# IXarea/LittleGAN

Measured on AMD Instinct MI355X. Metric: 128x128 CelebA-shaped images/sec (G+D+Adj step), higher is better.
Workload: dtype bf16; 1 GPU; C3: 128x128x3 synthetic CelebA, batch 256/GPU, bf16 MFMA conv/transposed-conv + Adjuster branch; global_batch=256, per_gpu_batch=256, image=128, cond_dim=40, parallelism=dp1, launch=eager launches

## Files before the change

### include/littlegan_hip.h

```cpp
#ifndef LITTLEGAN_HIP_H
#define LITTLEGAN_HIP_H
#include <stddef.h>

#ifdef __cplusplus
extern "C" {
#endif

#define LG_ABI_VERSION 1
#define LG_OK 0
#define LG_ERR_ARG (-1)
#define LG_ERR_LAUNCH (-2)
#define LG_ERR_UNSUPPORTED (-3)
#define LG_DT_F32 0
#define LG_DT_BF16 1

int lg_abi_version(void);
const char* lg_last_error(void);
const char* lg_last_kernel(void);
int lg_clear_kernel(void);

size_t lg_conv_pack_bytes(int cb, int cs, int dtype);
int lg_conv_pack(const float* w, void* pack, int cb, int cs, int dtype, void* stream);

int lg_conv2d_s2_fwd(const float* x, const void* pack, const float* bias, float* y, int B, int Hs, int Ws, int cb,
// ... 65 lines not shown
                               int B, void* stream);
int lg_instnorm_leaky_apply_z16_p(const void* z16, const void* partials, int nparts, const float* gamma, const float* beta,
                                  float* stats, const void* skip, int skip_is_bf16, float* y, void* y16, int B, long long L,
                                  int post_leaky, float alpha, void* stream);
int lg_instnorm_leaky_apply(const float* x, const float* stats, const float* skip, float* y, void* y16, int B,
                            long long L, int pre_leaky, int post_leaky, float alpha, void* stream);
int lg_instnorm_leaky_bwd(const float* x, const float* stats, const void* g, int g_is_bf16, float* dx, void* dx16,
                          float* dgamma, float* dbeta, void* workspace, size_t ws_bytes, int B, long long L,
                          int pre_leaky, int post_leaky, float alpha, int accumulate, void* stream);
size_t lg_instnorm_bwd_db_workspace_bytes(int B, long long L, int C);
int lg_instnorm_leaky_bwd_db(const float* x, const float* stats, const void* g, int g_is_bf16, float* dx, void* dx16,
                             float* dgamma, float* dbeta, float* db, int C, void* workspace, size_t ws_bytes, int B,
                             long long L, int pre_leaky, int post_leaky, float alpha, int accumulate, void* stream);
int lg_instnorm_leaky_apply_z16(const void* z16, const float* stats, const void* skip, int skip_is_bf16, float* y, void* y16,
                                int B, long long L, int pre_leaky, int post_leaky, float alpha, void* stream);
int lg_instnorm_leaky_bwd_z16(const void* z16, const float* stats, const void* g, int g_is_bf16, float* dx, void* dx16,
                              float* dgamma, float* dbeta, float* db, int C, void* workspace, size_t ws_bytes, int B,
                              long long L, int pre_leaky, int post_leaky, float alpha, int accumulate, void* stream);
int lg_instnorm_leaky_bwd_z16_p(const void* z16, const float* stats, const void* g, int g_is_bf16, float* dx, void* dx16,
                                float* dgamma, float* dbeta, float* db, int C, const void* partials, int nparts_in,
                                void* workspace, size_t ws_bytes, int B, long long L, int pre_leaky, int post_leaky, float alpha,
                                int accumulate, void* stream);
int lg_conv2d_s2_dgrad_nf(const void* dy16, const void* pack, void* dx16, int B, int Hs, int Ws, int cb, int cs,
                          const void* z16, const float* stats, float alpha, void* part, size_t part_bytes, int* nparts,
                          void* stream);
int lg_convT_s2_dgrad_nf(const void* dy16, const void* pack, void* dx16, int B, int Hs, int Ws, int cb, int cs,
                         const void* z16, const float* stats, float alpha, void* part, size_t part_bytes, int* nparts,
                         void* stream);

int lg_convT_s2_dgrad_bn_supported(int B, int Hs, int Ws, int cb, int cs);
int lg_convT_s2_dgrad_bn(const void* z16, const void* g16, const float* coef, float alpha, const void* pack, void* dx16,
                         int B, int Hs, int Ws, int cb, int cs, const void* zl16, const float* stats_l, float alpha_l,
                         void* part, size_t part_bytes, int* nparts, void* stream);
int lg_instnorm_bwd_coef(const float* stats, const void* partials, int nparts, float* coef, int B, long long L, void* stream);

int lg_dropout_key(long long* key, unsigned long long seed, unsigned long long key_offset, void* stream);
int lg_dropout_mask(const long long* key, int call, int level, int r0, int B, long long L, float rate, unsigned char* keep,
                    void* stream);
int lg_instnorm_leaky_apply_drop(const float* x, const float* stats, float* y, void* y16, int B, long long L, float alpha,
                                 const long long* key, int call, int level, int r0, float rate, void* stream);
int lg_instnorm_leaky_apply_z16_drop(const void* z16, const float* stats, float* y, void* y16, int B, long long L, float alpha,
                                     const long long* key, int call, int level, int r0, float rate, void* stream);
int lg_instnorm_leaky_apply_z16_p_drop(const void* z16, const void* partials, int nparts, const float* gamma, const float* beta,
                                       float* stats, float* y, void* y16, int B, long long L, float alpha, const long long* key,
                                       int call, int level, int r0, float rate, void* stream);
int lg_instnorm_leaky_bwd_drop(const float* x, const float* stats, const void* g, int g_is_bf16, float* dx, void* dx16,
                               float* dgamma, float* dbeta, float* db, int C, void* workspace, size_t ws_bytes, int B,
                               long long L, float alpha, int accumulate, const long long* key, int call, int level, int r0,
                               float rate, void* stream);
int lg_instnorm_leaky_bwd_z16_drop(const void* z16, const float* stats, const void* g, int g_is_bf16, float* dx, void* dx16,
                                   float* dgamma, float* dbeta, float* db, int C, const void* partials, int nparts_in,
                                   void* workspace, size_t ws_bytes, int B, long long L, float alpha, int accumulate,
                                   const long long* key, int call, int level, int r0, float rate, void* stream);

int lg_convT_s1_tanh_bwd_nf(const float* x, const void* x16, const float* dpre, const void* pack, void* dx16, float* dw,
                            float* db, void* workspace, size_t ws_bytes, int B, int H, int W, int cb, int cs, int accumulate,
                            int dtype, const void* z16, const float* stats, float alpha, void* part, size_t part_bytes,
                            int* nparts, void* stream);

int lg_dense_fwd(const float* x, const float* w, const float* bias, float* y, int B, int K, int N, void* stream);
int lg_dense_wgrad(const float* x, const float* dy, float* dw, float* db, int B, int K, int N, int accumulate,
                   void* stream);
int lg_dense_dgrad(const float* dy, const float* w, float* dx, int B, int K, int N, void* stream);
int lg_concat_cols(const float* a, int ka, const float* c, int kc, float* out, int B, void* stream);
int lg_adj_conditions(const float* first, const float* second, float* t, float* u, int B, int c, void* stream);
size_t lg_heads_fwd_workspace_bytes(int B, int K, int c);
// ... 80 lines not shown
```

### littlegan_amd/_lib.py

```python
from __future__ import annotations

import ctypes as C
import os

_HERE = os.path.dirname(os.path.abspath(__file__))
LIB_PATH = os.path.join(_HERE, "liblittlegan_hip.so")

DT_F32, DT_BF16 = 0, 1

P, I, L, F, Z = C.c_void_p, C.c_int, C.c_longlong, C.c_float, C.c_size_t

SIGNATURES = {
    "lg_abi_version": (I, []),
    "lg_last_error": (C.c_char_p, []),
    "lg_conv_pack_bytes": (Z, [I, I, I]),
    "lg_conv_pack": (I, [P, P, I, I, I, P]),
    "lg_conv2d_s2_fwd": (I, [P, P, P, P, I, I, I, I, I, I, P]),
    "lg_conv_stats_workspace_bytes": (Z, [I, I, I, I, I]),
    "lg_conv_fwd_stats_fused": (I, [I, I, I, I, I, I, I]),
    "lg_conv2d_s2_fwd_stats": (I, [P, P, P, P, P, P, I, I, I, I, I, I, P, Z, P, P]),
    "lg_conv2d_s2_dgrad_m16": (I, [P, P, P, P, P, I, I, I, I, I, I, P]),
    "lg_conv2d_s2_wgrad_m16": (I, [P, P, P, P, P, P, Z, I, I, I, I, I, I, I, P]),
    "lg_conv2d_s2_dgrad": (I, [P, P, P, I, I, I, I, I, I, P]),
    "lg_conv2d_s2_wgrad": (I, [P, P, P, P, Z, I, I, I, I, I, I, I, P]),
# ... 8 lines not shown
    "lg_convT_s1_tanh_bwd": (I, [P, P, P, P, P, P, P, Z, I, I, I, I, I, I, I, P]),
    "lg_convT_s1_bwd_workspace_bytes": (Z, [I, I, I, I, I, I]),
    "lg_n3_m16_supported": (I, [I, I, I, I, I]),
    "lg_convT_s1_tanh_fwd_m16": (I, [P, P, P, P, P, I, I, I, I, I, I, P]),
    "lg_conv2d_s2_fwd_stats_zn_supported": (I, [I, I, I, I, I, I]),
    "lg_conv2d_s2_fwd_stats_zn": (I, [P, P, F, P, P, P, I, I, I, I, I, I, P, Z, P, P]),
    "lg_convT_s1_tanh_fwd_z16_supported": (I, [I, I, I, I, I]),
    "lg_convT_s1_tanh_fwd_z16": (I, [P, P, F, P, P, P, I, I, I, I, I, I, P]),
    "lg_convT_s1_tanh_bwd_m16": (I, [P, P, P, P, P, P, P, P, P, Z, I, I, I, I, I, I, I, P]),
    "lg_bias_grad_workspace_bytes": (Z, [L, I]),
    "lg_bias_grad": (I, [P, P, P, Z, L, I, I, P]),
    "lg_bias_grad_m16": (I, [P, P, P, P, Z, L, I, I, P]),
    "lg_conv_halo_supported": (I, [I, I, I, I, I, I, I]),
    "lg_instnorm_workspace_bytes": (Z, [I, L]),
    "lg_instnorm_stats_stride": (I, []),
    "lg_instnorm_leaky_stats": (I, [P, P, P, P, P, Z, I, L, I, F, P]),
    "lg_instnorm_leaky_stats_z16": (I, [P, P, P, P, P, Z, I, L, I, F, P, P]),
    "lg_instnorm_stats_finalize": (I, [P, I, P, P, P, I, P]),
    "lg_instnorm_leaky_apply": (I, [P, P, P, P, P, I, L, I, I, F, P]),
    "lg_instnorm_leaky_bwd": (I, [P, P, P, I, P, P, P, P, P, Z, I, L, I, I, F, I, P]),
    "lg_instnorm_bwd_db_workspace_bytes": (Z, [I, L, I]),
    "lg_instnorm_leaky_bwd_db": (I, [P, P, P, I, P, P, P, P, P, I, P, Z, I, L, I, I, F, I, P]),
    "lg_last_kernel": (C.c_char_p, []),
    "lg_clear_kernel": (I, []),
    "lg_instnorm_leaky_apply_z16": (I, [P, P, P, I, P, P, I, L, I, I, F, P]),
    "lg_instnorm_leaky_apply_z16_p": (I, [P, P, I, P, P, P, P, I, P, P, I, L, I, F, P]),
    "lg_instnorm_leaky_bwd_z16": (I, [P, P, P, I, P, P, P, P, P, I, P, Z, I, L, I, I, F, I, P]),
    "lg_instnorm_leaky_bwd_z16_p": (I, [P, P, P, I, P, P, P, P, P, I, P, I, P, Z, I, L, I, I, F, I, P]),
    "lg_conv2d_s2_dgrad_nf": (I, [P, P, P, I, I, I, I, I, P, P, F, P, Z, P, P]),
    "lg_convT_s2_dgrad_nf": (I, [P, P, P, I, I, I, I, I, P, P, F, P, Z, P, P]),
    "lg_convT_s2_dgrad_bn_supported": (I, [I, I, I, I, I]),
    "lg_convT_s2_dgrad_bn": (I, [P, P, P, F, P, P, I, I, I, I, I, P, P, F, P, Z, P, P]),
    "lg_instnorm_bwd_coef": (I, [P, P, I, P, I, L, P]),
    "lg_dropout_key": (I, [P, L, L, P]),
    "lg_dropout_mask": (I, [P, I, I, I, I, L, F, P, P]),
    "lg_instnorm_leaky_apply_drop": (I, [P, P, P, P, I, L, F, P, I, I, I, F, P]),
    "lg_instnorm_leaky_apply_z16_drop": (I, [P, P, P, P, I, L, F, P, I, I, I, F, P]),
    "lg_instnorm_leaky_apply_z16_p_drop": (I, [P, P, I, P, P, P, P, P, I, L, F, P, I, I, I, F, P]),
    "lg_instnorm_leaky_bwd_drop": (I, [P, P, P, I, P, P, P, P, P, I, P, Z, I, L, F, I, P, I, I, I, F, P]),
    "lg_instnorm_leaky_bwd_z16_drop": (I, [P, P, P, I, P, P, P, P, P, I, P, I, P, Z, I, L, F, I, P, I, I, I, F, P]),
    "lg_convT_s1_tanh_bwd_nf": (I, [P, P, P, P, P, P, P, P, Z, I, I, I, I, I, I, I, P, P, F, P, Z, P, P]),
    "lg_dense_fwd": (I, [P, P, P, P, I, I, I, P]),
    "lg_dense_wgrad": (I, [P, P, P, P, I, I, I, I, P]),
    "lg_dense_dgrad": (I, [P, P, P, I, I, I, P]),
    "lg_concat_cols": (I, [P, I, P, I, P, I, P]),
    "lg_adj_conditions": (I, [P, P, P, P, I, I, P]),
    "lg_heads_fwd_workspace_bytes": (Z, [I, I, I]),
    "lg_heads_fwd": (I, [P, P, P, P, P, P, P, Z, I, I, I, P]),
    "lg_heads_dgrad": (I, [P, P, P, P, I, I, I, P]),
    "lg_heads_wgrad": (I, [P, P, P, P, P, P, I, I, I, I, P]),
    "lg_bce_heads_loss_fwd_bwd": (I, [P, P, F, F, F, P, P, I, I, I, P]),
    "lg_l1_workspace_bytes": (Z, []),
    "lg_l1_tanh_loss_fwd_bwd": (I, [P, P, P, P, P, P, Z, L, F, I, P]),
    "lg_clip_adam_update": (I, [P, P, P, P, L, P, F, F, F, F, F, F, P]),
    "lg_adam_advance": (I, [P, F, F, P]),
    "lg_axpby": (I, [P, P, F, F, L, P]),
    "lg_philox4x32": (I, [P, I, L, L, P]),
    "lg_randn": (I, [P, L, F, F, L, L, P]),
    "lg_augment_workspace_bytes": (Z, [I]),
    "lg_augment": (I, [P, P, I, I, I, P, F, F, F, F, L, L, P, Z, P]),
    "lg_fid_stats_workspace_bytes": (Z, [L, I]),
    "lg_fid_stats": (I, [P, L, I, P, P, P, Z, P]),
    "lg_fid_accum": (I, [P, L, I, P, P, P, P]),
    "lg_fid_finalize": (I, [P, P, P, L, I, P, P, P]),
    "lg_fid_gemm": (I, [P, P, P, I, P, P]),
    "lg_fid_distance_workspace_bytes": (Z, [I]),
# ... 65 lines not shown
```

### littlegan_amd/csrc/capi.hip

```cpp
#include <stdarg.h>
#include <stdio.h>
#include <stdlib.h>
#include "lg_common.h"
#include "../../include/littlegan_hip.h"

static thread_local char g_err[512] = "";

extern "C" void lg_set_error(const char* fmt, ...) {
  va_list ap;
  va_start(ap, fmt);
  vsnprintf(g_err, sizeof(g_err), fmt, ap);
  va_end(ap);
}
extern "C" const char* lg_last_error(void) { return g_err; }
static thread_local const char* g_kernel = "";
extern "C" void lg_note_kernel(const char* name) { g_kernel = name ? name : ""; }
extern "C" const char* lg_last_kernel(void) { return g_kernel; }
extern "C" int lg_clear_kernel(void) { g_kernel = ""; return LG_OK; }
extern "C" int lg_abi_version(void) { return LG_ABI_VERSION; }

extern "C" int lg_conv_igemm(int mode, int dtype, const float* src, const void* wpack, const float* bias, float* out,
                             int B, int Hm, int Wm, int Cs, int N, int act, int pstride, int ppad, void* stream);
extern "C" int lg_conv_igemm_ex(int mode, int dtype, const float* src, const void* src16, const void* wpack,
                                const float* bias, float* out, void* out16, int B, int Hm, int Wm, int Cs, int N, int act,
// ... 161 lines not shown
extern "C" int lg_convT_s2_dgrad_nf(const void* dy16, const void* pack, void* dx16, int B, int Hs, int Ws, int cb, int cs,
                                    const void* z16, const float* stats, float alpha, void* part, size_t part_bytes,
                                    int* nparts, void* stream) {
  LG_CHECK_ARG(dy16 && pack && dx16 && nparts, "lg_convT_s2_dgrad_nf: null pointer");
  *nparts = 0;
  if (cb != 3 && z16 && stats && part) {
    LgNormFuse nf{(const __bf16*)z16, stats, (double*)part, alpha, 0};
    const int rc = lg_conv_down3_nf_try(dy16, pack, nullptr, dx16, B, Hs, Ws, cb, cs, nullptr, 0, nparts, &nf, part_bytes, stream);
    if (rc != LG_ERR_UNSUPPORTED) return rc;
    *nparts = 0;
  }
  return lg_convT_s2_dgrad_m16(nullptr, dy16, pack, nullptr, dx16, B, Hs, Ws, cb, cs, LG_DT_BF16, stream);
}

extern "C" int lg_conv_down3_bn_supported(int B, int Hm, int Wm, int Cs, int N);
extern "C" int lg_conv_down3_bn_try(const void* z16, const void* g16, const float* bcoef, float alpha, const void* wpack, void* out16,
                                    int B, int Hm, int Wm, int Cs, int N, int* nparts_out, const LgNormFuse* nf, size_t nf_bytes,
                                    void* stream);
extern "C" int lg_convT_s2_dgrad_bn_supported(int B, int Hs, int Ws, int cb, int cs) {
  return cb != 3 ? lg_conv_down3_bn_supported(B, Hs, Ws, cb, cs) : 0;
}
extern "C" int lg_convT_s2_dgrad_bn(const void* z16, const void* g16, const float* coef, float alpha, const void* pack, void* dx16,
                                    int B, int Hs, int Ws, int cb, int cs, const void* zl16, const float* stats_l, float alpha_l,
                                    void* part, size_t part_bytes, int* nparts, void* stream) {
  LG_CHECK_ARG(z16 && g16 && coef && pack && dx16 && zl16 && stats_l && part && nparts, "lg_convT_s2_dgrad_bn: null pointer");
  *nparts = 0;
  LgNormFuse nf{(const __bf16*)zl16, stats_l, (double*)part, alpha_l, 0};
  const int rc = lg_conv_down3_bn_try(z16, g16, coef, alpha, pack, dx16, B, Hs, Ws, cb, cs, nparts, &nf, part_bytes, stream);
  if (rc == LG_ERR_UNSUPPORTED) lg_set_error("lg_convT_s2_dgrad_bn: shape B=%d %dx%d cb=%d cs=%d has no backward-normalising kernel "
                                             "(see lg_convT_s2_dgrad_bn_supported)", B, Hs, Ws, cb, cs);
  return rc;
}

extern "C" int lg_conv2d_s2_wgrad_m16(const float* x, const void* x16, const float* dy, const void* dy16, float* dw,
                                      void* workspace, size_t ws_bytes, int B, int Hs, int Ws, int cb, int cs,
                                      int accumulate, int dtype, void* stream) {
  return lg_conv_wgrad_m16(x, x16, dy, dy16, dw, workspace, ws_bytes, B, Hs, Ws, cb, cs, 2, 1, accumulate, dtype, stream);
}
extern "C" int lg_convT_s2_wgrad_m16(const float* x, const void* x16, const float* dy, const void* dy16, float* dw,
                                     void* workspace, size_t ws_bytes, int B, int Hs, int Ws, int cb, int cs,
                                     int accumulate, int dtype, void* stream) {
  return lg_conv_wgrad_m16(dy, dy16, x, x16, dw, workspace, ws_bytes, B, Hs, Ws, cb, cs, 2, 1, accumulate, dtype, stream);
}
extern "C" int lg_conv2d_s2_dgrad(const float* dy, const void* pack, float* dx, int B, int Hs, int Ws, int cb, int cs,
                                  int dtype, void* stream) {
  return run_up(dy, pack, nullptr, dx, B, Hs, Ws, cb, cs, dtype, stream);
}
extern "C" int lg_conv2d_s2_wgrad(const float* x, const float* dy, float* dw, void* workspace, size_t ws_bytes, int B,
                                  int Hs, int Ws, int cb, int cs, int accumulate, int dtype, void* stream) {
  return lg_conv_wgrad(x, dy, dw, workspace, ws_bytes, B, Hs, Ws, cb, cs, 2, 1, accumulate, dtype, stream);
}
extern "C" int lg_convT_s2_fwd(const float* x, const void* pack, const float* bias, float* y, int B, int Hs, int Ws,
                               int cb, int cs, int dtype, void* stream) {
  return run_up(x, pack, bias, y, B, Hs, Ws, cb, cs, dtype, stream);
}
extern "C" int lg_convT_s2_dgrad(const float* dy, const void* pack, float* dx, int B, int Hs, int Ws, int cb, int cs,
                                 int dtype, void* stream) {
  return run_down(dy, pack, nullptr, dx, B, Hs, Ws, cb, cs, dtype, stream);
}
extern "C" int lg_convT_s2_wgrad(const float* x, const float* dy, float* dw, void* workspace, size_t ws_bytes, int B,
                                 int Hs, int Ws, int cb, int cs, int accumulate, int dtype, void* stream) {
  return lg_conv_wgrad(dy, x, dw, workspace, ws_bytes, B, Hs, Ws, cb, cs, 2, 1, accumulate, dtype, stream);
}

extern "C" int lg_n3_m16_supported(int H, int W, int cb, int cs, int dtype) {
  return (dtype == LG_DT_BF16 && cb == 3 && lg_n3_enabled() && lg_n3_p16_supported(H, W, cs)) ? 1 : 0;
// ... 138 lines not shown
```

### littlegan_amd/csrc/n3_pgemm.hip

```cpp
#include <type_traits>
#include "lg_common.h"

#ifndef LG_P16_DBG
#define LG_P16_DBG 0
#endif
namespace {

constexpr int TS = 16;
constexpr int PR = 17;

__device__ __forceinline__ bf16x8 cvt8(const float* p) {
  const f32x4 a = *reinterpret_cast<const f32x4*>(p), b = *reinterpret_cast<const f32x4*>(p + 4);
  bf16x8 v;
  v[0] = (__bf16)a[0]; v[1] = (__bf16)a[1]; v[2] = (__bf16)a[2]; v[3] = (__bf16)a[3];
  v[4] = (__bf16)b[0]; v[5] = (__bf16)b[1]; v[6] = (__bf16)b[2]; v[7] = (__bf16)b[3];
  return v;
}
__device__ __forceinline__ bf16x8 zero8() {
  return __builtin_bit_cast(bf16x8, u32x4{0u, 0u, 0u, 0u});
}

template <int C>
__device__ __forceinline__ void load_bfrags(const float* __restrict__ w, int lane, bf16x8 (&bf)[5][C / 32]) {
  const int n = lane & 15, g = lane >> 4;
// ... 25 lines not shown
#pragma unroll
    for (int kh = 0; kh < KH; ++kh)
      af[i][kh] = ok ? *reinterpret_cast<const bf16x8*>(x16 + ((long long)(n * H + sy) * W + sx) * C + kh * 32 + g * 8) : zero8();
  }
  load_bfrags<C>(w, lane, bf);

  const int ly = threadIdx.x / TS, lx = threadIdx.x % TS;
  float acc[3] = {bias[0], bias[1], bias[2]};
#pragma unroll
  for (int ky = 0; ky < 5; ++ky) {
#pragma unroll
    for (int i = 0; i < MTW; ++i) {
      const int mt = wid + 4 * i;
      if (mt < NMT) {
        f32x4 c = {0.f, 0.f, 0.f, 0.f};
#pragma unroll
        for (int kh = 0; kh < KH; ++kh) c = __builtin_amdgcn_mfma_f32_16x16x32_bf16(af[i][kh], bf[ky][kh], c, 0, 0, 0);
#pragma unroll
        for (int e = 0; e < 4; ++e) sP[(mt * 16 + 4 * g + e) * PR + r] = c[e];
      }
    }
    __syncthreads();
#pragma unroll
    for (int kx = 0; kx < 5; ++kx) {
      const float* pp = sP + ((ly + 4 - ky) * HS + (lx + 4 - kx)) * PR + kx * 3;
      acc[0] += pp[0]; acc[1] += pp[1]; acc[2] += pp[2];
    }
    __syncthreads();
  }
  float* o = y + ((long long)(n * H + y0 + ly) * W + x0 + lx) * 3;
  o[0] = tanhf(acc[0]); o[1] = tanhf(acc[1]); o[2] = tanhf(acc[2]);
}

template <int C>
__global__ __launch_bounds__(256, 1) void up_p16_kernel(const __bf16* __restrict__ src16, const float* __restrict__ w,
                                                     float* __restrict__ out, int B, int H, int W) {
  constexpr int HS = TS + 2, NQ = HS * HS, NMT = (NQ + 15) / 16, MTW = (NMT + 3) / 4, KH = C / 32;
  __shared__ float sP[NMT * 16 * PR];
  const int lane = threadIdx.x & 63, wid = threadIdx.x >> 6, r = lane & 15, g = lane >> 4;
  const int tpx = W / TS, tpi = tpx * (H / TS), ntiles = B * tpi, G = gridDim.x;

  bf16x8 bf[5][KH];
  load_bfrags<C>(w, lane, bf);
  auto load_af = [&](int t, bf16x8 (&af)[MTW][KH]) {
    const int n = t / tpi, tt = t - n * tpi;
    const int y0 = (tt / tpx) * TS, x0 = (tt % tpx) * TS;
#pragma unroll
    for (int i = 0; i < MTW; ++i) {
      const int mt = wid + 4 * i, q = mt * 16 + r;
      const int sy = y0 - 1 + q / HS, sx = x0 - 1 + q % HS;
      const bool ok = q < NQ && (unsigned)sy < (unsigned)H && (unsigned)sx < (unsigned)W;
#pragma unroll
      for (int kh = 0; kh < KH; ++kh)
        af[i][kh] = (ok && !(LG_P16_DBG & 64)) ? *reinterpret_cast<const bf16x8*>(src16 + ((long long)(n * H + sy) * W + sx) * C + kh * 32 + g * 8) : zero8();
    }
  };
  const int ly = threadIdx.x / TS, lx = threadIdx.x % TS;
  auto compute = [&](int t, const bf16x8 (&af)[MTW][KH]) {
    const int n = t / tpi, tt = t - n * tpi;
    const int y0 = (tt / tpx) * TS, x0 = (tt % tpx) * TS;
    float acc[4][3];
#pragma unroll
    for (int k = 0; k < 4; ++k) { acc[k][0] = 0.f; acc[k][1] = 0.f; acc[k][2] = 0.f; }
#pragma unroll
    for (int ky = 0; ky < 5; ++ky) {
#pragma unroll
      for (int i = 0; i < MTW; ++i) {
        const int mt = wid + 4 * i;
        if (mt < NMT) {
          f32x4 c = {0.f, 0.f, 0.f, 0.f};
#pragma unroll
          for (int kh = 0; kh < KH; ++kh) c = __builtin_amdgcn_mfma_f32_16x16x32_bf16(af[i][kh], bf[ky][kh], c, 0, 0, 0);
#pragma unroll
          for (int e = 0; e < 4; ++e) {
            if constexpr (!(LG_P16_DBG & 32)) sP[(mt * 16 + 4 * g + e) * PR + r] = c[e];
            else if (c[e] == 12345.f) sP[(mt * 16 + 4 * g + e) * PR + r] = c[e];
          }
        }
      }
      if constexpr (!(LG_P16_DBG & 128)) __syncthreads();
      const int py = 1 - (ky & 1), dy = (py + 1 - ky) / 2;
#pragma unroll
      for (int kx = 0; kx < ((LG_P16_DBG & 16) ? 1 : 5); ++kx) {
        const int px = 1 - (kx & 1), dx = (px + 1 - kx) / 2;
        const float* pp = sP + ((ly + 1 + dy) * HS + (lx + 1 + dx)) * PR + kx * 3;
        acc[py * 2 + px][0] += pp[0]; acc[py * 2 + px][1] += pp[1]; acc[py * 2 + px][2] += pp[2];
      }
      if constexpr (!(LG_P16_DBG & 128)) __syncthreads();
    }
    const int yq = y0 + ly, xq = x0 + lx;
#pragma unroll
    for (int py = 0; py < 2; ++py) {
      float* o = out + ((long long)(n * 2 * H + 2 * yq + py) * 2 * W + 2 * xq) * 3;
#pragma unroll
      for (int px = 0; px < 2; ++px)
#pragma unroll
        for (int co = 0; co < 3; ++co) o[px * 3 + co] = acc[py * 2 + px][co];
    }
  };
  bf16x8 afA[MTW][KH], afB[MTW][KH];
  int t = blockIdx.x;
  if (t < ntiles) load_af(t, afA);
  for (; t < ntiles; t += 2 * G) {
    if (t + G < ntiles) load_af(t + G, afB);
    compute(t, afA);
    if (t + G < ntiles) {
      if (t + 2 * G < ntiles) load_af(t + 2 * G, afA);
      compute(t + G, afB);
    }
  }
}


template <int S, int N, bool OUT16, bool STATS, bool FUSE = false>
__global__ __launch_bounds__(256, 4) void patch_p16_kernel(const float* __restrict__ src, const float* __restrict__ w,
                                                        const float* __restrict__ bias, float* __restrict__ out,
                                                        __bf16* __restrict__ out16, double* __restrict__ spart, int B,
                                                        int H, int W, int pad, LgNormFuse nf = LgNormFuse{}) {
  static_assert(!FUSE || (OUT16 && !STATS), "norm-backward sums: bf16 data-gradient form only");
  constexpr bool CSPLIT = N == 64;
  constexpr int NWC = CSPLIT ? N / 2 : N;
  constexpr int NT = NWC / 16, HSIDE = S * (TS - 1) + 5, PW = (HSIDE + 2) & ~1, TROWS = HSIDE + 1, NKS = 4;
  constexpr int MTW = CSPLIT ? TS / 2 : TS / 4;
  constexpr bool HAS_BIAS = S == 2;
  __shared__ __attribute__((aligned(16))) bf16x4 tile[TROWS * PW];
  __shared__ __attribute__((aligned(16))) float cst[4][16 * NWC];
  __shared__ double sred[40];
  const int lane = threadIdx.x & 63, wid = __builtin_amdgcn_readfirstlane(threadIdx.x >> 6), r = lane & 15, g = lane >> 4;
  const int tpx = W / TS, tpi = tpx * (H / TS), ntiles = B * tpi;
  const int Hs = S * H, Ws = S * W;
  const int chw = CSPLIT ? (wid & 1) : 0, rw = CSPLIT ? (wid >> 1) : wid;

  bf16x8 bf[NKS][NT];
#pragma unroll
  for (int ks = 0; ks < NKS; ++ks)
#pragma unroll
    for (int nt = 0; nt < NT; ++nt) {
      bf16x8 v;
#pragma unroll
      for (int j = 0; j < 8; ++j) {
        const int kp = 32 * ks + 8 * g + j, ky = kp / 24, rem = kp - 24 * ky, kx = rem >> 2, c4 = rem & 3;
// ... 160 lines not shown

}

static int patch_grid(int ntiles, int per_cu) {
  static int cus = 0;
  if (!cus) {
    int dev = 0;
    hipDeviceProp_t pr;
    cus = 256;
    if (hipGetDevice(&dev) == hipSuccess && hipGetDeviceProperties(&pr, dev) == hipSuccess && pr.multiProcessorCount > 0) cus = pr.multiProcessorCount;
  }
  const int nb = per_cu * (cus < lg_grid_cus() ? cus : lg_grid_cus());
  return ntiles < nb ? ntiles : nb;
}

extern "C" int lg_n3_p16_supported(int H, int W, int C) { return (H % TS == 0 && W % TS == 0 && (C == 32 || C == 64)) ? 1 : 0; }

extern "C" int lg_n3_s1t_fwd_p16_try(const void* x16, const float* w, const float* bias, float* y, int B, int H, int W,
                                     int C, void* stream) {
  if (!lg_n3_p16_supported(H, W, C) || !x16 || !w || !bias) return LG_ERR_UNSUPPORTED;
  hipStream_t st = (hipStream_t)stream;
  const dim3 grid(B * (H / TS) * (W / TS));
  if (C == 32) hipLaunchKernelGGL(s1t_fwd_p16_kernel<32>, grid, dim3(256), 0, st, (const __bf16*)x16, w, bias, y, B, H, W);
  else hipLaunchKernelGGL(s1t_fwd_p16_kernel<64>, grid, dim3(256), 0, st, (const __bf16*)x16, w, bias, y, B, H, W);
  LG_CHECK_LAUNCH("lg_n3_s1t_fwd_p16");
  lg_note_kernel("s1t_fwd_p16_kernel");
  return LG_OK;
}

extern "C" int lg_n3_up_p16_try(const void* src16, const float* w, float* out, int B, int H, int W, int C, void* stream) {
  if (!lg_n3_p16_supported(H, W, C) || !src16 || !w) return LG_ERR_UNSUPPORTED;
  hipStream_t st = (hipStream_t)stream;
  const dim3 grid(patch_grid(B * (H / TS) * (W / TS), 2));
  if (C == 32) hipLaunchKernelGGL(up_p16_kernel<32>, grid, dim3(256), 0, st, (const __bf16*)src16, w, out, B, H, W);
  else hipLaunchKernelGGL(up_p16_kernel<64>, grid, dim3(256), 0, st, (const __bf16*)src16, w, out, B, H, W);
  LG_CHECK_LAUNCH("lg_n3_up_p16");
  lg_note_kernel("up_p16_kernel");
  return LG_OK;
}

extern "C" int lg_n3_conv1_p16_supported(int H, int W, int N) { return (H % TS == 0 && W % TS == 0 && N == 64) ? 1 : 0; }

extern "C" int lg_n3_conv1_fwd_p16_try(const float* img, const float* w, const float* bias, float* z, void* z16, int B, int H,
                                       int W, int N, void* spart, size_t spart_bytes, int* nparts, void* stream) {
  if (nparts) *nparts = 0;
  if (H % TS || W % TS || N != 64 || !img || !w || (!z && !z16)) return LG_ERR_UNSUPPORTED;
  hipStream_t st = (hipStream_t)stream;
  const int tpi = (H / TS) * (W / TS), ntiles = B * tpi;
  const dim3 grid(patch_grid(ntiles, 4));
  const bool stats = spart && nparts && (size_t)B * tpi * 3 * sizeof(double) <= spart_bytes;
  if (z16) {
    if (stats) hipLaunchKernelGGL((patch_p16_kernel<2, 64, true, true>), grid, dim3(256), 0, st, img, w, bias, nullptr, (__bf16*)z16, (double*)spart, B, H, W, 1);
    else hipLaunchKernelGGL((patch_p16_kernel<2, 64, true, false>), grid, dim3(256), 0, st, img, w, bias, nullptr, (__bf16*)z16, nullptr, B, H, W, 1);
  } else if (stats) hipLaunchKernelGGL((patch_p16_kernel<2, 64, false, true>), grid, dim3(256), 0, st, img, w, bias, z, nullptr, (double*)spart, B, H, W, 1);
  else hipLaunchKernelGGL((patch_p16_kernel<2, 64, false, false>), grid, dim3(256), 0, st, img, w, bias, z, nullptr, nullptr, B, H, W, 1);
  LG_CHECK_LAUNCH("lg_n3_conv1_fwd_p16");
  lg_note_kernel("patch_p16_kernel<2,64>");
  if (stats) *nparts = tpi;
  return LG_OK;
}

extern "C" int lg_n3_s1_dgrad_p16_nf_try(const float* dpre, const float* w, float* dx, void* dx16, int B, int H, int W, int N,
                                         const LgNormFuse* nf, size_t nf_bytes, int* nparts_out, void* stream);
extern "C" int lg_n3_s1_dgrad_p16_try(const float* dpre, const float* w, float* dx, void* dx16, int B, int H, int W, int N,
                                      void* stream) {
  return lg_n3_s1_dgrad_p16_nf_try(dpre, w, dx, dx16, B, H, W, N, nullptr, 0, nullptr, stream);
}
extern "C" int lg_n3_s1_dgrad_p16_nf_try(const float* dpre, const float* w, float* dx, void* dx16, int B, int H, int W, int N,
                                         const LgNormFuse* nf, size_t nf_bytes, int* nparts_out, void* stream) {
  if (nparts_out) *nparts_out = 0;
// ... 19 lines not shown
```

### littlegan_amd/model.py

```python
from __future__ import annotations

import math
import zlib
from typing import Dict, List, Optional

import torch

from . import ops
from ._lib import DT_BF16, DT_F32


def _dtype_of(args) -> int:
    name = getattr(args, "mfma_dtype", "f32")
    if name not in ("f32", "bf16"):
        raise ValueError(f"mfma_dtype must be 'f32' or 'bf16', got {name!r}")
    return DT_BF16 if name == "bf16" else DT_F32


def _device_of(args):
    return torch.device(getattr(args, "device", "cuda"))


def _glorot(shape, gen, device):
    if len(shape) == 2:
# ... 31 lines not shown
    def weights(self) -> List[torch.Tensor]:
        return [self._w[n] for n in self._names]

    def own_items(self):
        return [(n, self._w[n]) for n in self._names]

    def grad(self, name) -> Optional[torch.Tensor]:
        return self._g.get(name)


class _ConvStack(_Module):

    def __init__(self, args, chans):
        super().__init__(args)
        self.chans = chans
        self._packs: List[Optional[torch.Tensor]] = [None] * 4
        self._pack_version = -1
        self.version = 0
        for i, (cb, cs) in enumerate(chans, 1):
            self._add(f"conv{i}.kernel", (5, 5, cb, cs), "kernel")
            self._add(f"conv{i}.bias", (self._bias_dim(cb, cs),), "zeros")
            self._add(f"norm{i}.gamma", (1,), "ones")
            self._add(f"norm{i}.beta", (1,), "zeros")

    def packs(self):
        if self._pack_version != self.version:
            for i, (cb, cs) in enumerate(self.chans):
                self._packs[i] = ops.conv_pack(self._w[f"conv{i + 1}.kernel"], cb, cs, self.dtype, out=self._packs[i])
            self._pack_version = self.version
        return self._packs


class Encoder(_ConvStack):

    def __init__(self, args):
        cf = args.conv_filter
        chans, cin = [], args.image_channel
        for i in range(1, 5):
            chans.append((cin, cf[4 - i]))
            cin = cf[4 - i]
        super().__init__(args, chans)

    @staticmethod
    def _bias_dim(cb, cs):
        return cs

    def __call__(self, inputs, ctx: Optional[dict] = None, tails=None, keep_maps: bool = True, top_only: bool = False,
                 drop: Optional[ops.Drop] = None):
        x = inputs
        a = self.args.leaky_alpha
        packs = self.packs()
        outs = []
        saved = []
        m16 = self.dtype == DT_BF16
        x16 = None
        if top_only and (tails is not None or not m16 or (drop is not None and drop.active)):
            top_only = False
        drops = [drop.at(level=i, r0=0) for i in range(1, 5)] if drop is not None else None
        raw = None
        for i, (cb, cs) in enumerate(self.chans, 1):
            gm, bt = self._w[f"norm{i}.gamma"], self._w[f"norm{i}.beta"]
            Bn, Hn, Wn = (x if x is not None else x16 if x16 is not None else raw[0]).shape[:3]
            skip_apply = (top_only and i < 4 and
                          ops.conv2d_s2_fwd_stats_zn_supported(Bn, Hn // 2, Wn // 2, cs, self.chans[i][1], self.dtype))
            if raw is not None:
                z, st = ops.conv2d_s2_fwd_stats_zn(raw[0], raw[1], a, packs[i - 1], self._w[f"conv{i}.bias"], cs, self.dtype, gm, bt)
# ... 29 lines not shown
        return outs

    def backward(self, ctx, g_last, need_wgrad: bool, need_input_grad: bool, rows: Optional[slice] = None,
                 wgrad_levels=None):
        a = self.args.leaky_alpha
        packs = self.packs()
        drops = ctx.get("enc_drop")
        r0 = 0
        if drops is not None and rows is not None:
            r0, _, step = rows.indices(ctx["enc"][0][1].shape[0])
            if step != 1:
                raise ValueError("Encoder.backward: contiguous row ranges only")
        masked = drops is not None and drops[0].active
        g_h = g_last
        levels = set(range(1, 5)) if (need_wgrad and wgrad_levels is None) else (set(wgrad_levels or ()) if need_wgrad else set())
        lowest = 1 if need_input_grad else (min(levels) if levels else 5)
        any_wgrad = need_wgrad
        nfp = None
        for i in range(4, lowest - 1, -1):
            need_wgrad = any_wgrad and i in levels
            cb, cs = self.chans[i - 1]
            x, z, st, x16 = ctx["enc"][i - 1]
            if need_wgrad and x is None and x16 is None:
                raise ValueError("Encoder.backward: this context was recorded with top_only=True (no normalised inputs kept): "
                                 "it cannot give weight gradients")
            if rows is not None:
                z, st = z[rows], st[rows]
                x = x[rows] if x is not None else None
                x16 = x16[rows] if x16 is not None else None
            dgm = self._g[f"norm{i}.gamma"] if need_wgrad else None
            dbt = self._g[f"norm{i}.beta"] if need_wgrad else None
            want_dx = i > lowest or (i == 1 and need_input_grad)
            m16 = self.dtype == DT_BF16
            if cb != 3:
                dz16 = torch.empty(z.shape, dtype=torch.bfloat16, device=z.device) if m16 else None
                drop32 = (m16 and (not need_wgrad or x16 is not None) and
                          (not want_dx or ops.conv_halo_supported(1, self.dtype, z.shape[0], z.shape[1], z.shape[2], cs, cb)))
            else:
                drop32 = m16 and ops.n3_m16_supported(z.shape[1], z.shape[2], cb, cs, self.dtype)
                dz16 = torch.empty(z.shape, dtype=torch.bfloat16, device=z.device) if drop32 else None
            dz = ops.instnorm_bwd(z, st, g_h, dgm, dbt, 0, 1, a, out16=dz16, want_f32=not drop32,
                                  db=self._g[f"conv{i}.bias"] if need_wgrad else None,
                                  partials=nfp, drop=drops[i - 1].at(r0=r0) if drops is not None else None)
            nfp = None
            if need_wgrad:
                ops.conv2d_s2_wgrad(x, dz, self._g[f"conv{i}.kernel"], False, self.dtype, x16=x16, dy16=dz16)
            if not want_dx:
                g_h = None
            elif m16 and i > 1 and drop32 and i - 1 >= lowest and not masked:
                zl, stl = ctx["enc"][i - 2][1], ctx["enc"][i - 2][2]
                if rows is not None:
                    zl, stl = zl[rows], stl[rows]
                g_h, nfp = ops.conv2d_s2_dgrad(None, packs[i - 1], cb, self.dtype, dy16=dz16, out_bf16=True, fuse=(zl, stl, a))
            else:
                g_h = ops.conv2d_s2_dgrad(dz, packs[i - 1], cb, self.dtype, dy16=dz16, out_bf16=(self.dtype == DT_BF16 and i > 1))
        return g_h if need_input_grad else None

    def backward_recorded(self, ctx, g_last):
        a = self.args.leaky_alpha
        packs = self.packs()
        rec = {}
        g_h = g_last
        for i in range(4, 0, -1):
            cb, _ = self.chans[i - 1]
            _, z, st, _ = ctx["enc"][i - 1]
            dz = ops.gp_norm_bwd(z, st, self._w[f"norm{i}.gamma"], g_h, a)
# ... 449 lines not shown
```

### littlegan_amd/ops.py

```python
from __future__ import annotations

import torch

from . import _lib
from ._lib import DT_BF16, DT_F32, check

_WS = {}
_WS_RETIRED = []
_WS_PINNED = False
NSTAT = 8


class Profile:
    enabled = False
    records = []
    after_conv = None

    @classmethod
    def start(cls):
        cls.records = []
        cls.enabled = True

    @classmethod
    def stop(cls):
# ... 236 lines not shown


def instnorm_bwd_coef(z16, stats, partials):
    B = z16.shape[0]
    _chk(stats, (B, NSTAT), "stats")
    if tuple(z16.shape) != partials.shape:
        raise ValueError(f"instnorm_bwd_coef: partial sums were produced for shape {partials.shape}, got {tuple(z16.shape)}")
    coef = torch.empty(B, 8, dtype=torch.float32, device=z16.device)
    check(_lib.load().lg_instnorm_bwd_coef(_p(stats), _p(partials.buf), int(partials.nparts), _p(coef), B, z16.numel() // B, _stream()),
          "lg_instnorm_bwd_coef")
    return coef


def convT_s2_dgrad_bn(z16, g16, coef, alpha, pack, cs, fuse):
    import ctypes
    B, H, W, cb = z16.shape
    _chk16(z16, z16, "z16")
    _chk16(g16, z16, "g16")
    if tuple(g16.shape) != tuple(z16.shape):
        raise ValueError("convT_s2_dgrad_bn: z16 and g16 must have the same shape")
    _chk(coef, (B, 8), "coef")
    if not convT_s2_dgrad_bn_supported(B, H // 2, W // 2, cb, cs, DT_BF16):
        raise ValueError(f"convT_s2_dgrad_bn: unsupported shape B={B} {H // 2}x{W // 2} cb={cb} cs={cs}")
    out = torch.empty(B, H // 2, W // 2, cs, dtype=torch.bfloat16, device=z16.device)
    zl, stl, alpha_l, ws, npo = _nf_args(fuse, B, False, H // 2, W // 2, cs, z16.device)
    e0 = _pb()
    check(_lib.load().lg_convT_s2_dgrad_bn(_p(z16), _p(g16), _p(coef), float(alpha), _p(pack), _p(out), B, H // 2, W // 2, cb, cs,
                                          _p(zl), _p(stl), alpha_l, _p(ws), ws.numel(), ctypes.addressof(npo), _stream()),
          "lg_convT_s2_dgrad_bn")
    _pe(e0, "conv_igemm_down", 50.0 * B * (H // 2) * (W // 2) * cb * cs)
    if npo.value <= 0:
        raise _lib.LittleGanHipError("lg_convT_s2_dgrad_bn returned no partial sums")
    return out, NormPartials(ws, npo.value, alpha_l, out.shape)


def convT_s2_wgrad(x, dy, dw, accumulate, dtype, x16=None, dy16=None):
    return _wgrad("lg_convT_s2_wgrad_m16", dy, x, dw, accumulate, dtype, swap=True, big16=dy16, small16=x16)


def n3_m16_supported(H, W, cb, cs, dtype):
    return bool(_lib.load().lg_n3_m16_supported(H, W, cb, cs, dtype))


def convT_s1_tanh_fwd(x, pack, bias, cb, dtype, out=None, x16=None):
    t = x if x is not None else x16
    B, H, W, cs = t.shape
    if x is not None:
        _chk(x, name="x")
    if x16 is not None:
        _chk16(x16, t, "x16")
    if out is None:
        out = torch.empty(B, H, W, cb, dtype=torch.float32, device=t.device)
    _chk(out, (B, H, W, cb), "out")
    _chk(bias, (cb,), "bias")
    e0 = _pb()
    check(_lib.load().lg_convT_s1_tanh_fwd_m16(_p(x), _p(x16), _p(pack), _p(bias), _p(out), B, H, W, cb, cs, dtype,
                                               _stream()), "lg_convT_s1_tanh_fwd_m16")
    _pe(e0, "conv_igemm_s1t_n3", 50.0 * B * H * W * cb * cs)
    return out


def convT_s1_tanh_fwd_z16_supported(H, W, cb, cs, dtype):
    return bool(_lib.load().lg_convT_s1_tanh_fwd_z16_supported(H, W, cb, cs, dtype))


def convT_s1_tanh_fwd_z16(z16, stats, alpha, pack, bias, cb, dtype, out=None):
# ... 866 lines not shown
```

Baseline: 23890 images/sec.

## Fuse instance-norm backward into level-1 encoder input-gradient conv kernel

Adds a BWDNORM variant of the 3-channel up_p16 dgrad kernel. It applies the instance-norm/leaky backward on the fly to the next tile's activations while the current tile computes. The encoder's level-1 backward, used when only the input gradient is needed, calls it with precomputed coefficients and skips the separate instnorm_bwd pass and its bf16 dz buffer. The variant also uses buffer loads with hardware OOB handling, stages filter fragments in LDS to cut register use, and raises occupancy to two blocks per CU. It adds interleaved work per filter-row pass, which could lengthen the critical path.

Result: no change. 24030 images/sec (median of 6 runs) (+0.6%).

```diff
diff --git a/include/littlegan_hip.h b/include/littlegan_hip.h
--- a/include/littlegan_hip.h
+++ b/include/littlegan_hip.h
@@ -121,6 +121,9 @@
 int lg_convT_s2_dgrad_bn(const void* z16, const void* g16, const float* coef, float alpha, const void* pack, void* dx16,
                          int B, int Hs, int Ws, int cb, int cs, const void* zl16, const float* stats_l, float alpha_l,
                          void* part, size_t part_bytes, int* nparts, void* stream);
+int lg_conv2d_s2_dgrad_bn_supported(int B, int Hs, int Ws, int cb, int cs);
+int lg_conv2d_s2_dgrad_bn(const void* z16, const void* g16, const float* coef, float alpha, const void* pack, float* dx,
+                          int B, int Hs, int Ws, int cb, int cs, void* stream);
 int lg_instnorm_bwd_coef(const float* stats, const void* partials, int nparts, float* coef, int B, long long L, void* stream);
 
 int lg_dropout_key(long long* key, unsigned long long seed, unsigned long long key_offset, void* stream);
diff --git a/littlegan_amd/_lib.py b/littlegan_amd/_lib.py
--- a/littlegan_amd/_lib.py
+++ b/littlegan_amd/_lib.py
@@ -64,6 +64,8 @@
     "lg_convT_s2_dgrad_bn_supported": (I, [I, I, I, I, I]),
     "lg_convT_s2_dgrad_bn": (I, [P, P, P, F, P, P, I, I, I, I, I, P, P, F, P, Z, P, P]),
     "lg_instnorm_bwd_coef": (I, [P, P, I, P, I, L, P]),
+    "lg_conv2d_s2_dgrad_bn_supported": (I, [I, I, I, I, I]),
+    "lg_conv2d_s2_dgrad_bn": (I, [P, P, P, F, P, P, I, I, I, I, I, P]),
     "lg_dropout_key": (I, [P, L, L, P]),
     "lg_dropout_mask": (I, [P, I, I, I, I, L, F, P, P]),
     "lg_instnorm_leaky_apply_drop": (I, [P, P, P, P, I, L, F, P, I, I, I, F, P]),
diff --git a/littlegan_amd/csrc/capi.hip b/littlegan_amd/csrc/capi.hip
--- a/littlegan_amd/csrc/capi.hip
+++ b/littlegan_amd/csrc/capi.hip
@@ -217,6 +217,22 @@
   return rc;
 }
 
+extern "C" int lg_n3_up_p16_bn_try(const void* z16, const void* g16, const float* coef, float alpha, const float* w, float* out,
+                                   int B, int H, int W, int C, void* stream);
+extern "C" int lg_conv2d_s2_dgrad_bn_supported(int B, int Hs, int Ws, int cb, int cs) {
+  return (B > 0 && cb == 3 && lg_n3_enabled() && lg_n3_p16_supported(Hs, Ws, cs) && (long long)Hs * Ws * cs * 2 < (1ll << 31)) ? 1 : 0;
+}
+extern "C" int lg_conv2d_s2_dgrad_bn(const void* z16, const void* g16, const float* coef, float alpha, const void* pack, float* dx,
+                                     int B, int Hs, int Ws, int cb, int cs, void* stream) {
+  LG_CHECK_ARG(z16 && g16 && coef && pack && dx, "lg_conv2d_s2_dgrad_bn: null pointer");
+  int rc = LG_ERR_UNSUPPORTED;
+  if (lg_conv2d_s2_dgrad_bn_supported(B, Hs, Ws, cb, cs))
+    rc = lg_n3_up_p16_bn_try(z16, g16, coef, alpha, raw_pack(pack, cb, cs, LG_DT_BF16), dx, B, Hs, Ws, cs, stream);
+  if (rc == LG_ERR_UNSUPPORTED) lg_set_error("lg_conv2d_s2_dgrad_bn: shape B=%d %dx%d cb=%d cs=%d has no backward-normalising kernel "
+                                             "(see lg_conv2d_s2_dgrad_bn_supported)", B, Hs, Ws, cb, cs);
+  return rc;
+}
+
 extern "C" int lg_conv2d_s2_wgrad_m16(const float* x, const void* x16, const float* dy, const void* dy16, float* dw,
                                       void* workspace, size_t ws_bytes, int B, int Hs, int Ws, int cb, int cs,
                                       int accumulate, int dtype, void* stream) {
diff --git a/littlegan_amd/csrc/n3_pgemm.hip b/littlegan_amd/csrc/n3_pgemm.hip
--- a/littlegan_amd/csrc/n3_pgemm.hip
+++ b/littlegan_amd/csrc/n3_pgemm.hip
@@ -81,45 +81,116 @@
   o[0] = tanhf(acc[0]); o[1] = tanhf(acc[1]); o[2] = tanhf(acc[2]);
 }
 
-template <int C>
-__global__ __launch_bounds__(256, 1) void up_p16_kernel(const __bf16* __restrict__ src16, const float* __restrict__ w,
-                                                     float* __restrict__ out, int B, int H, int W) {
+template <int C, bool BN = false>
+__global__ __launch_bounds__(256, BN ? 2 : 1) void up_p16_kernel(const __bf16* __restrict__ src16, const float* __restrict__ w,
+                                                     float* __restrict__ out, int B, int H, int W,
+                                                     const __bf16* __restrict__ g16 = nullptr, const float* __restrict__ coef = nullptr,
+                                                     float alpha = 0.f) {
   constexpr int HS = TS + 2, NQ = HS * HS, NMT = (NQ + 15) / 16, MTW = (NMT + 3) / 4, KH = C / 32;
+  static_assert(!BN || MTW == 6, "BWDNORM: six m-tiles per wave over five filter-row passes");
   __shared__ float sP[NMT * 16 * PR];
-  const int lane = threadIdx.x & 63, wid = threadIdx.x >> 6, r = lane & 15, g = lane >> 4;
+  const int lane = threadIdx.x & 63, wid = BN ? __builtin_amdgcn_readfirstlane(threadIdx.x >> 6) : threadIdx.x >> 6, r = lane & 15, g = lane >> 4;
   const int tpx = W / TS, tpi = tpx * (H / TS), ntiles = B * tpi, G = gridDim.x;
 
   bf16x8 bf[5][KH];
   load_bfrags<C>(w, lane, bf);
-  auto load_af = [&](int t, bf16x8 (&af)[MTW][KH]) {
+  __shared__ bf16x8 sB[BN ? 5 * KH * 64 : 1];
+  if constexpr (BN) {
+    if (wid == 0) {
+#pragma unroll
+      for (int ky = 0; ky < 5; ++ky)
+#pragma unroll
+        for (int kh = 0; kh < KH; ++kh) sB[(ky * KH + kh) * 64 + lane] = bf[ky][kh];
+    }
+    __syncthreads();
+  }
+  auto piece = [&](int t, int i) -> long long {
     const int n = t / tpi, tt = t - n * tpi;
     const int y0 = (tt / tpx) * TS, x0 = (tt % tpx) * TS;
+    const int mt = wid + 4 * i, q = mt * 16 + r;
+    const int sy = y0 - 1 + q / HS, sx = x0 - 1 + q % HS;
+    const bool ok = q < NQ && (unsigned)sy < (unsigned)H && (unsigned)sx < (unsigned)W;
+    return ok ? ((long long)(n * H + sy) * W + sx) * C + g * 8 : -1;
+  };
+  constexpr unsigned OOB = 0x80000000u;
+  const int sample_elems = H * W * C;
+  unsigned rel[BN ? MTW : 1], edge = 0;
+  (void)rel;
+  if constexpr (BN) {
 #pragma unroll
     for (int i = 0; i < MTW; ++i) {
-      const int mt = wid + 4 * i, q = mt * 16 + r;
-      const int sy = y0 - 1 + q / HS, sx = x0 - 1 + q % HS;
-      const bool ok = q < NQ && (unsigned)sy < (unsigned)H && (unsigned)sx < (unsigned)W;
-#pragma unroll
-      for (int kh = 0; kh < KH; ++kh)
-        af[i][kh] = (ok && !(LG_P16_DBG & 64)) ? *reinterpret_cast<const bf16x8*>(src16 + ((long long)(n * H + sy) * W + sx) * C + kh * 32 + g * 8) : zero8();
+      const int q = (wid + 4 * i) * 16 + r, qy = q / HS, qx = q % HS;
+      rel[i] = (unsigned)(((qy * W + qx) * C + g * 8) * 2);
+      edge |= (qx == 0 ? 1u << i : 0u) | (qx == HS - 1 ? 0x100u << i : 0u) | (q >= NQ ? 0x10000u << i : 0u);
+    }
+  }
+  auto boff = [&](int t, int i) -> unsigned {
+    const int tt = t % tpi;
+    const int y0 = (tt / tpx) * TS, x0 = (tt % tpx) * TS;
+    const unsigned m = (t < 0 || (LG_P16_DBG & 64)) ? 0xffffffu : (0x3f0000u | (x0 == 0 ? 0x3fu : 0u) | (x0 + TS == W ? 0x3f00u : 0u));
+    const unsigned o = (unsigned)(((y0 - 1) * W + (x0 - 1)) * C * 2) + rel[i];
+    return (edge & m & (0x10101u << i)) ? OOB : o;
+  };
+  auto bload = [&](const __bf16* base, int t, int i, bf16x8 (&v)[KH]) {
+    const __amdgpu_buffer_rsrc_t rs = __builtin_amdgcn_make_buffer_rsrc(
+        const_cast<__bf16*>(base + (long long)((t < 0 ? 0 : t) / tpi) * sample_elems), 0, sample_elems * 2, 0x00027000);
+    const unsigned o = boff(t, i);
+#pragma unroll
+    for (int kh = 0; kh < KH; ++kh) v[kh] = __builtin_bit_cast(bf16x8, __builtin_amdgcn_raw_buffer_load_b128(rs, o + kh * 64u, 0, 0));
+  };
+  auto load_af = [&](int t, bf16x8 (&af)[MTW][KH]) {
+#pragma unroll
+    for (int i = 0; i < MTW; ++i) {
+      if constexpr (BN) bload(src16, t, i, af[i]);
+      else {
+        const long long o = piece(t, i);
+#pragma unroll
+        for (int kh = 0; kh < KH; ++kh)
+          af[i][kh] = (o >= 0 && !(LG_P16_DBG & 64)) ? *reinterpret_cast<const bf16x8*>(src16 + o + kh * 32) : zero8();
+      }
+    }
+  };
+  auto load_g = [&](int t, int i, bf16x8 (&gq)[KH]) { bload(g16, t, i, gq); };
+  auto read_coef = [&](int t) {
+    const lg_const_f32p sp = lg_as_const(coef + (long long)((t < 0 ? 0 : t) / tpi) * 8);
+    LgBwdCoef co;
+    co.mu = lg_uniform(sp[0]); co.mul = lg_uniform(sp[1]); co.a = lg_uniform(sp[2]); co.b = lg_uniform(sp[3]);
+    co.m1 = lg_uniform(sp[4]); co.m2 = lg_uniform(sp[5]); co.m1l = lg_uniform(sp[6]); co.m2l = lg_uniform(sp[7]);
+    return co;
+  };
+  auto norm_mt = [&](int t, int i, bf16x8 (&af)[MTW][KH], const bf16x8 (&gq)[KH], const LgBwdCoef& co) {
+    const bool inside = boff(t, i) < (unsigned)(sample_elems * 2);
+#pragma unroll
+    for (int kh = 0; kh < KH; ++kh) {
+      const u32x4 dn = lg_bwdnorm8(__builtin_bit_cast(u32x4, af[i][kh]), __builtin_bit_cast(u32x4, gq[kh]), co, alpha);
+      af[i][kh] = inside ? __builtin_bit_cast(bf16x8, dn) : zero8();
     }
   };
   const int ly = threadIdx.x / TS, lx = threadIdx.x % TS;
-  auto compute = [&](int t, const bf16x8 (&af)[MTW][KH]) {
+  auto compute = [&](int t, const bf16x8 (&af)[MTW][KH], int tn, bf16x8 (&afn)[MTW][KH]) {
     const int n = t / tpi, tt = t - n * tpi;
     const int y0 = (tt / tpx) * TS, x0 = (tt % tpx) * TS;
     float acc[4][3];
 #pragma unroll
     for (int k = 0; k < 4; ++k) { acc[k][0] = 0.f; acc[k][1] = 0.f; acc[k][2] = 0.f; }
+    bf16x8 gq[KH];
+    LgBwdCoef co{};
+    (void)gq; (void)co;
+    if constexpr (BN) {
+      co = read_coef(tn); load_g(tn, 0, gq);
+    }
 #pragma unroll
     for (int ky = 0; ky < 5; ++ky) {
+      bf16x8 bk[KH];
+#pragma unroll
+      for (int kh = 0; kh < KH; ++kh) bk[kh] = BN ? sB[(ky * KH + kh) * 64 + lane] : bf[ky][kh];
 #pragma unroll
       for (int i = 0; i < MTW; ++i) {
         const int mt = wid + 4 * i;
         if (mt < NMT) {
           f32x4 c = {0.f, 0.f, 0.f, 0.f};
 #pragma unroll
-          for (int kh = 0; kh < KH; ++kh) c = __builtin_amdgcn_mfma_f32_16x16x32_bf16(af[i][kh], bf[ky][kh], c, 0, 0, 0);
+          for (int kh = 0; kh < KH; ++kh) c = __builtin_amdgcn_mfma_f32_16x16x32_bf16(af[i][kh], bk[kh], c, 0, 0, 0);
 #pragma unroll
           for (int e = 0; e < 4; ++e) {
             if constexpr (!(LG_P16_DBG & 32)) sP[(mt * 16 + 4 * g + e) * PR + r] = c[e];
@@ -128,6 +199,9 @@
         }
       }
       if constexpr (!(LG_P16_DBG & 128)) __syncthreads();
+      if constexpr (BN) {
+        norm_mt(tn, ky, afn, gq, co); load_g(tn, ky + 1, gq);
+      }
       const int py = 1 - (ky & 1), dy = (py + 1 - ky) / 2;
 #pragma unroll
       for (int kx = 0; kx < ((LG_P16_DBG & 16) ? 1 : 5); ++kx) {
@@ -137,6 +211,9 @@
       }
       if constexpr (!(LG_P16_DBG & 128)) __syncthreads();
     }
+    if constexpr (BN) {
+      norm_mt(tn, 5, afn, gq, co);
+    }
     const int yq = y0 + ly, xq = x0 + lx;
 #pragma unroll
     for (int py = 0; py < 2; ++py) {
@@ -144,18 +221,28 @@
 #pragma unroll
       for (int px = 0; px < 2; ++px)
 #pragma unroll
-        for (int co = 0; co < 3; ++co) o[px * 3 + co] = acc[py * 2 + px][co];
+        for (int co3 = 0; co3 < 3; ++co3) o[px * 3 + co3] = acc[py * 2 + px][co3];
     }
   };
   bf16x8 afA[MTW][KH], afB[MTW][KH];
   int t = blockIdx.x;
-  if (t < ntiles) load_af(t, afA);
+  if (t < ntiles) {
+    load_af(t, afA);
+    if constexpr (BN) {
+      const LgBwdCoef co = read_coef(t);
+      bf16x8 gq[KH];
+#pragma unroll
+      for (int i = 0; i < MTW; ++i) { load_g(t, i, gq); norm_mt(t, i, afA, gq, co); }
+    }
+  }
   for (; t < ntiles; t += 2 * G) {
-    if (t + G < ntiles) load_af(t + G, afB);
-    compute(t, afA);
-    if (t + G < ntiles) {
-      if (t + 2 * G < ntiles) load_af(t + 2 * G, afA);
-      compute(t + G, afB);
+    const bool n1 = t + G < ntiles;
+    if (n1) load_af(t + G, afB);
+    compute(t, afA, (BN && n1) ? t + G : -1, afB);
+    if (n1) {
+      const bool n2 = t + 2 * G < ntiles;
+      if (n2) load_af(t + 2 * G, afA);
+      compute(t + G, afB, (BN && n2) ? t + 2 * G : -1, afA);
     }
   }
 }
@@ -382,10 +469,23 @@
   if (!lg_n3_p16_supported(H, W, C) || !src16 || !w) return LG_ERR_UNSUPPORTED;
   hipStream_t st = (hipStream_t)stream;
   const dim3 grid(patch_grid(B * (H / TS) * (W / TS), 2));
-  if (C == 32) hipLaunchKernelGGL(up_p16_kernel<32>, grid, dim3(256), 0, st, (const __bf16*)src16, w, out, B, H, W);
-  else hipLaunchKernelGGL(up_p16_kernel<64>, grid, dim3(256), 0, st, (const __bf16*)src16, w, out, B, H, W);
+  if (C == 32) hipLaunchKernelGGL((up_p16_kernel<32>), grid, dim3(256), 0, st, (const __bf16*)src16, w, out, B, H, W, nullptr, nullptr, 0.f);
+  else hipLaunchKernelGGL((up_p16_kernel<64>), grid, dim3(256), 0, st, (const __bf16*)src16, w, out, B, H, W, nullptr, nullptr, 0.f);
   LG_CHECK_LAUNCH("lg_n3_up_p16");
   lg_note_kernel("up_p16_kernel");
+  return LG_OK;
+}
+
+extern "C" int lg_n3_up_p16_bn_try(const void* z16, const void* g16, const float* coef, float alpha, const float* w, float* out,
+                                   int B, int H, int W, int C, void* stream) {
+  if (!lg_n3_p16_supported(H, W, C) || !z16 || !g16 || !coef || !w) return LG_ERR_UNSUPPORTED;
+  if ((long long)H * W * C * 2 >= (1ll << 31)) return LG_ERR_UNSUPPORTED;
+  hipStream_t st = (hipStream_t)stream;
+  const dim3 grid(patch_grid(B * (H / TS) * (W / TS), 2));
+  if (C == 32) hipLaunchKernelGGL((up_p16_kernel<32, true>), grid, dim3(256), 0, st, (const __bf16*)z16, w, out, B, H, W, (const __bf16*)g16, coef, alpha);
+  else hipLaunchKernelGGL((up_p16_kernel<64, true>), grid, dim3(256), 0, st, (const __bf16*)z16, w, out, B, H, W, (const __bf16*)g16, coef, alpha);
+  LG_CHECK_LAUNCH("lg_n3_up_p16_bn");
+  lg_note_kernel("up_p16_kernel<BWDNORM>");
   return LG_OK;
 }
 
diff --git a/littlegan_amd/model.py b/littlegan_amd/model.py
--- a/littlegan_amd/model.py
+++ b/littlegan_amd/model.py
@@ -87,6 +87,8 @@
 
 
 class Encoder(_ConvStack):
+
+    fuse_level1_bwdnorm = True
 
     def __init__(self, args):
         cf = args.conv_filter
@@ -182,6 +184,14 @@
             dbt = self._g[f"norm{i}.beta"] if need_wgrad else None
             want_dx = i > lowest or (i == 1 and need_input_grad)
             m16 = self.dtype == DT_BF16
+            if (self.fuse_level1_bwdnorm and i == 1 and want_dx and not need_wgrad and nfp is not None and not masked and m16
+                    and z.dtype == torch.bfloat16 and g_h.dtype == torch.bfloat16
+                    and ops.conv2d_s2_dgrad_bn_supported(z.shape[0], z.shape[1], z.shape[2], cb, cs, self.dtype)
+                    and ops.conv2d_s2_dgrad_bn_pays(z.shape[0], z.shape[1], z.shape[2])):
+                coef = ops.instnorm_bwd_coef(z, st, nfp)
+                g_h = ops.conv2d_s2_dgrad_bn(z, g_h, coef, a, packs[0], cb)
+                nfp = None
+                continue
             if cb != 3:
                 dz16 = torch.empty(z.shape, dtype=torch.bfloat16, device=z.device) if m16 else None
                 drop32 = (m16 and (not need_wgrad or x16 is not None) and
diff --git a/littlegan_amd/ops.py b/littlegan_amd/ops.py
--- a/littlegan_amd/ops.py
+++ b/littlegan_amd/ops.py
@@ -292,6 +292,33 @@
     if npo.value <= 0:
         raise _lib.LittleGanHipError("lg_convT_s2_dgrad_bn returned no partial sums")
     return out, NormPartials(ws, npo.value, alpha_l, out.shape)
+
+
+def conv2d_s2_dgrad_bn_supported(B, Hs, Ws, cb, cs, dtype):
+    return dtype == DT_BF16 and bool(_lib.load().lg_conv2d_s2_dgrad_bn_supported(B, Hs, Ws, cb, cs))
+
+
+def conv2d_s2_dgrad_bn_pays(B, Hs, Ws):
+    return B * (Hs // 16) * (Ws // 16) > 2 * int(_lib.load().lg_grid_cus())
+
+
+def conv2d_s2_dgrad_bn(z16, g16, coef, alpha, pack, cb, out=None):
+    B, Hs, Ws, cs = z16.shape
+    _chk16(z16, z16, "z16")
+    _chk16(g16, z16, "g16")
+    if tuple(g16.shape) != tuple(z16.shape):
+        raise ValueError("conv2d_s2_dgrad_bn: z16 and g16 must have the same shape")
+    _chk(coef, (B, 8), "coef")
+    if not conv2d_s2_dgrad_bn_supported(B, Hs, Ws, cb, cs, DT_BF16):
+        raise ValueError(f"conv2d_s2_dgrad_bn: unsupported shape B={B} {Hs}x{Ws} cb={cb} cs={cs}")
+    if out is None:
+        out = torch.empty(B, 2 * Hs, 2 * Ws, cb, dtype=torch.float32, device=z16.device)
+    _chk(out, (B, 2 * Hs, 2 * Ws, cb), "out")
+    e0 = _pb()
+    check(_lib.load().lg_conv2d_s2_dgrad_bn(_p(z16), _p(g16), _p(coef), float(alpha), _p(pack), _p(out), B, Hs, Ws, cb, cs, _stream()),
+          "lg_conv2d_s2_dgrad_bn")
+    _pe(e0, "conv_igemm_up_n3", 50.0 * B * Hs * Ws * cb * cs)
+    return out
 
 
 def convT_s2_wgrad(x, dy, dw, accumulate, dtype, x16=None, dy16=None):
```
